# gnosisguild/pvw-rs

Measured on AMD Instinct MI355X. Metric: parties/s for n-party encrypt (pvw::crypto::encrypt); achieved HBM GB/s vs peak, higher is better.
Workload: dtype u64

## Files before the change

### pvw_rs_amd/csrc/pvw_capi.hip

```cpp
#include <hip/hip_runtime.h>

#include <algorithm>
#include <atomic>
#include <cmath>
#include <cstdio>
#include <cstring>
#include <functional>
#include <map>
#include <mutex>
#include <string>
#include <thread>
#include <vector>

#include "../../include/pvw_hip.h"
#include "pvw_arith.h"
#include "pvw_bignum.h"
#include "pvw_chacha.h"
#include "pvw_decode.h"
#include "pvw_kernels.h"
#if PVW_TUNING
#include "../../include/pvw_hip_tuning.h"
#endif

using namespace pvw;
// ... 138 lines not shown
  const bool by_kernel = stream_capturing(s);
  for (const Workspace::Span& sp : w->secrets) {
    hipError_t e = hipSuccess;
    if (!sp.cleared) e = by_kernel && sp.bytes % 8 == 0 ? launch_wipe_words((u64*)sp.p, sp.bytes / 8, s) : hipMemsetAsync(sp.p, 0, sp.bytes, s);
    if (e != hipSuccess) rc = e;
  }
  w->wiped = w->secrets;
  w->secrets.clear();
  return rc;
}

struct pvw_ctx {
  u32 n, k, l, L;
  std::vector<u64> moduli, psi;
  float variance;
  u64 b1, b2;
  u32 num_cus = 256;
  u32 xm_bytes = 8;
  int device;
  u32 party_lo, party_hi, c1_lo, c1_hi;
  BigInt Q, halfQ, delta, delta_pow;
  std::vector<BigInt> crt_qi;
  std::vector<u64> crt_inv;
  std::vector<Mod> mods;
  std::vector<u64> tw, itw, linv, ghat, gpow;
  bool roots_locked = false;
  std::vector<u64> dec_words;
  DecodeTables dec_host{};
  DecodeTables dec_dev{};
  void* d_dec = nullptr;

  std::atomic<bool> dev_ready{false};
  void* d_tables = nullptr;
  DevTables dt{};
  u64* dA = nullptr;
  u64* dB = nullptr;
  u64* xmA = nullptr;
  u64* xmB = nullptr;
  bool xm_valid = false;
  u64* pkA = nullptr;
  u64* pkB = nullptr;
  u32* pk_flag = nullptr;
  u32 pk_width = 0;
  bool pkA_valid = false, pkB_valid = false;
  bool pk_wide = false;
  u32 pk_nomem_calls = 0;
  bool crs_loaded = false;
  u32 num_keys = 0;
  hipStream_t stream = nullptr;

  std::mutex mu, init_mu;
  std::vector<Workspace*> pool;
  std::map<void*, Workspace*> async_ws;

  bool profiling = false;
  std::vector<ProfRec> prof;
  std::map<std::string, std::pair<double, uint64_t>> prof_acc;

  u32 rowsA() const { return c1_hi - c1_lo; }
  u32 rowsB() const { return party_hi - party_lo; }
  u32 R() const { return 128 / l; }
  size_t poly() const { return (size_t)L * l; }
  size_t tiled_words(u32 rows) const { return (size_t)((rows + R() - 1) / R()) * L * k * 128; }
};

struct ProfScope {
  pvw_ctx* c;
  hipStream_t s;
  ProfRec rec;
  bool on;
  ProfScope(pvw_ctx* c_, const char* name, hipStream_t s_) : c(c_), s(s_), on(c_->profiling) {
    if (on) {
      rec.name = name;
      hipEventCreate(&rec.a);
      hipEventCreate(&rec.b);
      hipEventRecord(rec.a, s);
    }
  }
  ~ProfScope() {
    if (on) {
      hipEventRecord(rec.b, s);
      std::lock_guard<std::mutex> g(c->mu);
      c->prof.push_back(rec);
    }
  }
};

static void build_tables(pvw_ctx* c) {
  const u32 L = c->L, l = c->l, bits = ilog2(l);
  c->tw.assign((size_t)L * l, 0);
  c->itw.assign((size_t)L * l, 0);
  c->linv.assign(L, 0);
  c->gpow.assign((size_t)L * l, 0);
  c->ghat.assign((size_t)L * l, 0);
  for (u32 i = 0; i < L; ++i) {
    const Mod& m = c->mods[i];
    u64 psi = c->psi[i], ipsi = powmod(psi, m.q - 2, m);
    for (u32 x = 0; x < l; ++x) {
      c->tw[(size_t)i * l + x] = powmod(psi, bitrev32(x, bits), m);
      c->itw[(size_t)i * l + x] = powmod(ipsi, bitrev32(x, bits), m);
    }
    c->linv[i] = powmod(l, m.q - 2, m);
    u64 dm = c->delta.mod_small(m.q), p = 1;
    for (u32 j = 0; j < l; ++j) {
      c->gpow[(size_t)i * l + j] = p;
      p = mulmod(p, dm, m);
    }
    std::vector<u64> g(c->gpow.begin() + (size_t)i * l, c->gpow.begin() + (size_t)(i + 1) * l);
    host_ntt_forward(g.data(), l, &c->tw[(size_t)i * l], m);
    std::copy(g.begin(), g.end(), c->ghat.begin() + (size_t)i * l);
  }
}

static double correctness_bound(double n, double k, double l, double b1, double b2) {
  double first = b2 * std::sqrt(n * l) * (1.0 + std::sqrt(n));
  double second = 2.0 * b1 * k * l;
  double third = 14.0 * b1 * std::sqrt(n * k * l);
  return first + second + third;
}
// ... 119 lines not shown
  char* p = (char*)c->d_tables;
  auto put = [&](const void* src, size_t n) -> const void* {
    const void* at = p;
    hipMemcpy(p, src, n, hipMemcpyHostToDevice);
    p += n;
    return at;
  };
  c->dt.mods = (const Mod*)put(c->mods.data(), L * sizeof(Mod));
  c->dt.min_q_bits = 64;
  c->dt.max_q_bits = 0;
  for (u32 i = 0; i < L; ++i) {
    u32 bits = 0;
    for (u64 q = c->mods[i].q; q; q >>= 1) ++bits;
    if (bits < c->dt.min_q_bits) c->dt.min_q_bits = bits;
    if (bits > c->dt.max_q_bits) c->dt.max_q_bits = bits;
  }
  c->dt.tw = (const u64*)put(c->tw.data(), L * l * 8);
  c->dt.itw = (const u64*)put(c->itw.data(), L * l * 8);
  c->dt.ghat = (const u64*)put(c->ghat.data(), L * l * 8);
  c->dt.gpow = (const u64*)put(c->gpow.data(), L * l * 8);
  c->dt.linv = (const u64*)put(c->linv.data(), L * 8);
  auto shoup = [&](const std::vector<u64>& src, size_t per_limb) {
    std::vector<u64> out(src.size());
    for (size_t i = 0; i < src.size(); ++i) out[i] = shoup_precompute(src[i], c->moduli[i / per_limb]);
    return out;
  };
  std::vector<u64> twp = shoup(c->tw, l), itwp = shoup(c->itw, l), ghatp = shoup(c->ghat, l),
                   gpowp = shoup(c->gpow, l), linvp = shoup(c->linv, 1);
  c->dt.twp = (const u64*)put(twp.data(), L * l * 8);
  c->dt.itwp = (const u64*)put(itwp.data(), L * l * 8);
  c->dt.ghatp = (const u64*)put(ghatp.data(), L * l * 8);
  c->dt.gpowp = (const u64*)put(gpowp.data(), L * l * 8);
  c->dt.linvp = (const u64*)put(linvp.data(), L * 8);
  if (!c->d_dec) PVW_HIP(hipMalloc(&c->d_dec, c->dec_words.size() * 8));
  PVW_HIP(hipMemcpy(c->d_dec, c->dec_words.data(), c->dec_words.size() * 8, hipMemcpyHostToDevice));
  {
    const u64* hb = c->dec_words.data();
    const u64* db = (const u64*)c->d_dec;
    DecodeTables d = c->dec_host;
    auto mv = [&](const u64* hp) { return db + (hp - hb); };
    d.mods = c->dt.mods;
    d.Q = mv(d.Q); d.halfQ = mv(d.halfQ); d.qi = mv(d.qi); d.inv = mv(d.inv); d.invp = mv(d.invp); d.pow64 = mv(d.pow64);
    d.dmod = mv(d.dmod); d.dmodp = mv(d.dmodp); d.delta = mv(d.delta); d.dpow = mv(d.dpow); d.half_dpow = mv(d.half_dpow);
    d.dpow_n = mv(d.dpow_n); d.td_n = mv(d.td_n);
    d.pow64T = mv(d.pow64T); d.td = mv(d.td); d.mu_td = mv(d.mu_td); d.mu_dp = mv(d.mu_dp); d.gar = mv(d.gar); d.sc = mv(d.sc); d.dpm = mv(d.dpm);
    c->dec_dev = d;
  }
  PVW_HIP(hipDeviceSynchronize());
  return PVW_OK;
}

static int32_t ensure_device(pvw_ctx* c) {
  if (c->dev_ready) {
    PVW_HIP(hipSetDevice(c->device));
    return PVW_OK;
  }
  std::lock_guard<std::mutex> init_guard(c->init_mu);
  if (c->dev_ready) {
    PVW_HIP(hipSetDevice(c->device));
    return PVW_OK;
  }
  int count = 0;
  if (hipGetDeviceCount(&count) != hipSuccess || count == 0)
    return fail(PVW_ERR_INTERNAL, "no HIP device available: the PVW hot path has no CPU fallback");
  if (c->device < 0) {
    int cur = 0;
// ... 411 lines not shown
    c->crt_inv.push_back(powmod(qi.mod_small(c->moduli[i]), c->moduli[i] - 2, c->mods[i]));
  }
  build_tables(c);
  build_decode_tables(c);
  {
    u32 maxbits = 0;
    for (u64 q : c->moduli) {
      u32 bits = 0;
      for (; q; q >>= 1) ++bits;
      if (bits > maxbits) maxbits = bits;
    }
    c->pk_width = packed_width(maxbits, c->k, c->l);
  }
  *out = c;
  return PVW_OK;
}

int32_t pvw_ctx_destroy(pvw_ctx* c) {
  if (!c) return PVW_OK;
  if (c->dev_ready) {
    hipSetDevice(c->device);
    hipDeviceSynchronize();
    for (auto& r : c->prof) { hipEventDestroy(r.a); hipEventDestroy(r.b); }
    for (Workspace* w : c->pool) ws_free(w);
    for (auto& kv : c->async_ws) ws_free(kv.second);
    hipFree(c->dA);
    hipFree(c->dB);
    hipFree(c->xmA);
    hipFree(c->xmB);
    hipFree(c->pkA);
    hipFree(c->pkB);
    hipFree(c->pk_flag);
    hipFree(c->d_tables);
    hipFree(c->d_dec);
    if (c->stream) hipStreamDestroy(c->stream);
  }
  delete c;
  return PVW_OK;
}

int32_t pvw_ctx_get_roots(const pvw_ctx* c, uint64_t* psi_out) {
  if (!c || !psi_out) return fail(PVW_ERR_INVALID_PARAMETERS, "NULL argument");
  memcpy(psi_out, c->psi.data(), c->L * 8);
  return PVW_OK;
}

int32_t pvw_ctx_set_roots(pvw_ctx* c, const uint64_t* psi) {
  if (!c || !psi) return fail(PVW_ERR_INVALID_PARAMETERS, "NULL argument");
  if (c->roots_locked)
    return fail(PVW_ERR_CONTEXT, "roots must be set before any device operation");
  for (u32 i = 0; i < c->L; ++i)
    if (psi[i] >= c->moduli[i] || powmod(psi[i], c->l, c->mods[i]) != c->moduli[i] - 1)
      return fail(PVW_ERR_INVALID_PARAMETERS, "psi is not a primitive 2l-th root of unity");
  c->psi.assign(psi, psi + c->L);
  build_tables(c);
  return PVW_OK;
}

static int32_t export_big(const BigInt& v, uint64_t* words, size_t cap, size_t* nwords) {
  if (!nwords) return fail(PVW_ERR_INVALID_PARAMETERS, "NULL argument");
  *nwords = v.mag.size();
  if (words) {
    if (cap < v.mag.size()) return fail(PVW_ERR_INSUFFICIENT_DATA, "word buffer too small");
    memcpy(words, v.mag.data(), v.mag.size() * 8);
  }
  return PVW_OK;
// ... 1203 lines not shown
      pb.njobs = fused_e2 ? 2 : 3;
      pb.reps = cnt;
      ProfScope ps(c, "prologue", s);
      PVW_HIP(launch_prologue(pb, c->dt, L, l, s));
    }
    u64* c1g = d_c1 + d0 * rA * P;
    u64* c2g = d_c2 + d0 * rB * P;
    const bool last = d0 + nv == D;
    if (use_gemm) {
      {
        ProfScope ps(c, "vec_digits", s);
        PVW_HIP(launch_vec_digits(vh, (size_t)k * P, w->yd, w->sy, nv, k, L, l, c->dt, s, 0, 0, c->xm_bytes));
      }
      ProfScope ps(c, "gemm_digits", s);
      GemmSection a{c->xmA, c1g, c1g, w->gtmpA, rA, 0, 0}, b{c->xmB, c2g, c2g, w->gtmpB, rB, 0, 0};
      std::vector<GemmErrSource> es;
      if (fused_e2) {
        for (u32 v0 = 0; v0 < nv; v0 += PVW_MAX_PROLOGUE_KEYS) {
          GemmErrSource e{};
          e.span = (nv - v0) < PVW_MAX_PROLOGUE_KEYS ? (nv - v0) : PVW_MAX_PROLOGUE_KEYS;
          keys.from(d0 + v0).fill(e, e.span);
          e.key_v = 1;
          e.domain = DOM_E2; e.index0 = c->party_lo; e.index_row = 1; e.index_v = 0; e.bound = c->b2;
          e.scalars = gsc + c->party_lo; e.scalar_v = c->n;
          es.push_back(e);
        }
        b.addend = nullptr;
      }
      if (rs && last) {
        GemmSection& fin = rB ? b : a;
        fin.rnd_ctr = &rs->counter;
        fin.rnd_adv = D;
      }
      PVW_HIP(launch_gemm_digits(a, b, w->yd, w->sy, c->dt, k, L, l, nv, (size_t)rA * P, (size_t)rB * P, s, nullptr, fused_e2 ? es.data() : nullptr, c->xm_bytes));
    } else {
      ProfScope ps(c, "mac_rows_multi", s);
      MacSection a(c->dA, c1g, c1g, rA), b(c->dB, c2g, c2g, rB);
      MultiVec mv{vh, (size_t)k * P, (size_t)rA * P, (size_t)rB * P, nv};
      if (rs && last) {
        a.rnd_ctr = &rs->counter;
        a.rnd_adv = D;
      }
      PVW_HIP(launch_mac_rows_multi(a, b, mv, c->dt, k, L, l, s));
    }
  }
  if (out_repr == PVW_REPR_POWER) {
    ProfScope ps(c, "intt", s);
    PVW_HIP(launch_ntt(d_c1, D * rA, true, c->dt, L, l, s));
    PVW_HIP(launch_ntt(d_c2, D * rB, true, c->dt, L, l, s));
  }
  return PVW_OK;
}

static int32_t encrypt_multi_checks(pvw_ctx* c, size_t D, size_t per_dealer, uint32_t out_repr) {
  PVW_TRY(check_repr(out_repr));
  if (D == 0) return fail(PVW_ERR_INVALID_PARAMETERS, "no dealers");
  if (per_dealer != c->n) {
    char buf[96];
    snprintf(buf, sizeof buf, "Dealer provided %zu shares but needs %u", per_dealer, c->n);
    return fail(PVW_ERR_INVALID_PARAMETERS, buf);
  }
  if (c->num_keys < c->party_hi)
    return fail(PVW_ERR_INVALID_PARAMETERS, "Global public key is not complete (missing party keys)");
  if (!c->crs_loaded) return fail(PVW_ERR_CRS, "CRS not loaded");
  int32_t ok = 0;
  pvw_ctx_verify_correctness_condition(c, &ok);
  if (!ok) return fail(PVW_ERR_INVALID_PARAMETERS, "Parameters do not satisfy correctness condition - decryption may fail");
// ... 1397 lines not shown
  sc.secret(w, r_small0, r_tmp);
  const u32 nchunks = (b - a + chunk - 1) / chunk;
  PVW_TRY(ws_aux(w, 2 * (size_t)nchunks + 2));
  auto upload = [&](u32 ci, hipStream_t st) -> int32_t {
    const u32 q0 = a + ci * chunk, cn = (b - q0) < chunk ? (b - q0) : chunk;
    const size_t wd = (size_t)cn * k * l;
    i64* dst = d_small2[ci & 1];
    PVW_HIP(hipMemcpyAsync(dst, sk + (size_t)(q0 - lo) * k * l, wd * 8, hipMemcpyHostToDevice, st));
    if (ek) PVW_HIP(hipMemcpyAsync(dst + (size_t)chunk * k * l, ek + (size_t)(q0 - lo) * k * l, wd * 8, hipMemcpyHostToDevice, st));
    return PVW_OK;
  };
  PVW_TRY(upload(0, s));
  PVW_HIP(launch_untile(c->dA, d_api, k, 0, k, L, l, false, c->dt, s));
  PVW_HIP(launch_vec_digits(d_api, P, d_yd, d_sy, k, k, L, l, c->dt, s, l, (size_t)k * P));
  for (u32 ci = 0; ci < nchunks; ++ci) {
    const u32 p0 = a + ci * chunk;
    const u32 cnt = (b - p0) < chunk ? (b - p0) : chunk;
    i64* d_small = d_small2[ci & 1];
    if (ci > 0) PVW_HIP(hipStreamWaitEvent(s, w->events[2 * ci], 0));
    ProfScope ps(c, "keygen", s);
    GemmSection ga{d_xm, d_erow, d_erow, d_tmp, cnt, 0, 0}, gb{nullptr, nullptr, nullptr, nullptr, 0, 0, 0};
    ga.tiled_out = c->dB;
    ga.tiled_row0 = p0 - c->party_lo;
    ga.tiled_swap = 1;
    ga.row_stride = (size_t)k * P;
    if (direct) {
      PVW_HIP(launch_shat_mftile(d_small, d_xm, cnt, k, L, l, c->dt, s));
      GemmErrSource es{};
      if (ek) { es.explicit_coeffs = d_small + (size_t)chunk * k * l; es.coef_row = k; es.coef_v = 1; }
      else es.key[0] = make_key(seed);
      es.domain = DOM_EKEY; es.index0 = p0 * k; es.index_row = k; es.index_v = 1; es.bound = c->b1;
      ga.addend = nullptr;
      ga.out = nullptr;
      PVW_HIP(launch_gemm_digits(ga, gb, d_yd, d_sy, c->dt, k, L, l, k, P, 0, s, &es));
    } else {
      PrologueBatch pb{};
      if (seed) pb.key[0] = make_key(seed);
      PrologueJob& js = pb.job[0];
      PrologueJob& je = pb.job[1];
      js.sj.count = k; js.explicit_coeffs = d_small; js.rep_coeffs = (size_t)k * l;
      js.out = d_srow; js.stride_poly = P; js.stride_limb = l; js.rep_out = (size_t)k * P;
      je.sj.kind = SAMPLE_UNIFORM; je.sj.domain = DOM_EKEY; je.sj.index0 = p0 * k; je.sj.count = k; je.sj.bound = c->b1;
      je.rep_index0 = k;
      if (ek) { je.explicit_coeffs = d_small + (size_t)chunk * k * l; je.rep_coeffs = (size_t)k * l; }
      je.out = d_erow; je.stride_poly = P; je.stride_limb = l; je.rep_out = (size_t)k * P;
      pb.njobs = 2;
      pb.reps = cnt;
      PVW_HIP(launch_prologue(pb, c->dt, L, l, s));
      PVW_HIP(hipMemsetAsync(d_xm, 0, xm_words(cnt, k, L, l) * 8, s));
      PVW_HIP(launch_mftile(d_srow, false, d_xm, cnt, k, L, l, s));
      PVW_HIP(launch_gemm_digits(ga, gb, d_yd, d_sy, c->dt, k, L, l, k, P, 0, s));
    }
    PVW_HIP(hipEventRecord(w->events[2 * ci + 1], s));
    if (ci + 1 < nchunks) {
      if (ci >= 1) PVW_HIP(hipStreamWaitEvent(w->aux, w->events[2 * (ci - 1) + 1], 0));
      PVW_TRY(upload(ci + 1, w->aux));
      PVW_HIP(hipEventRecord(w->events[2 * ci + 2], w->aux));
    }
  }
  return PVW_OK;
}

static int32_t keygen_transposed(pvw_ctx* c, Workspace* w, u32 a, u32 b, u32 lo, const int64_t* sk, const int64_t* ek,
                                 const uint8_t* seed, bool use_gemm) {
  const u32 k = c->k, l = c->l, L = c->L;
  const size_t P = c->poly();
  hipStream_t s = w->stream;
// ... 520 lines not shown
```

### pvw_rs_amd/csrc/pvw_gemm.hip

```cpp
#include <hip/hip_runtime.h>

#include "pvw_arith.h"
#include "pvw_chacha.h"
#include "pvw_decode.h"
#include "pvw_kernels.h"
#include "pvw_dev.h"

namespace pvw {

__global__ __launch_bounds__(64) void mfma_i8_probe_kernel(const signed char* __restrict__ A,
                                                            const signed char* __restrict__ B, int* __restrict__ Cm) {
  const u32 l = threadIdx.x, r = l & 31, h = l >> 5;
  union { v4i32 v; signed char b[16]; } fa, fb;
#pragma unroll
  for (int j = 0; j < 16; ++j) {
    fa.b[j] = A[r * 32 + 16 * h + j];
    fb.b[j] = B[(16 * h + j) * 32 + r];
  }
  v16i32 acc = {};
  acc = __builtin_amdgcn_mfma_i32_32x32x32_i8(fa.v, fb.v, acc, 0, 0, 0);
#pragma unroll
  for (int g = 0; g < 16; ++g) Cm[((g & 3) + 8 * (g >> 2) + 4 * h) * 32 + r] = acc[g];
}


template <int ELL>
__global__ __launch_bounds__(256) void mftile_kernel(const u64* __restrict__ src, u32 src_is_tiled,
                                                      u64* __restrict__ XM, u32 rows, u32 k, u32 L) {
  constexpr int R = 128 / ELL;
  const size_t tid = (size_t)blockIdx.x * blockDim.x + threadIdx.x;
  if (tid >= (size_t)rows * k * L) return;
  const u32 limb = tid % L;
  const u32 j = (tid / L) % k;
  const u32 row = tid / ((size_t)L * k);
  const u64* p = src_is_tiled ? src + (((size_t)(row / R) * L + limb) * k + j) * 128 + (row % R) * ELL
                              : src + tid * ELL;
  const u32 RT = ((rows + PVW_GEMM_ROWS_PER_WG - 1) / PVW_GEMM_ROWS_PER_WG) * (PVW_GEMM_ROWS_PER_WG / 32), JB = (k + 3) / 4;
  const u32 rt = row >> 5, m = row & 31, jb = j >> 2, h = (j >> 1) & 1, e = j & 1;
#pragma unroll
// ... 780 lines not shown
    for (int sl = 0; sl < ELL; ++sl) { a[sl] = signed_residue(c[sl], m); x[sl] = in[sl]; }
    if (limb + 1 < limb_end) load_tmp(limb + 1);
    ntt_forward<ELL>(a, t.tw + (size_t)limb * ELL, t.twp + (size_t)limb * ELL, m);
    if (es.scalars) {
      const u64 mr = signed_residue(scalar, m);
      const u64* g = t.ghat + (size_t)limb * ELL;
      const u64* gp = t.ghatp + (size_t)limb * ELL;
#pragma unroll
      for (int sl = 0; sl < ELL; ++sl) a[sl] = addmod(a[sl], mulmod_shoup(mr, g[sl], gp[sl], m.q), m.q);
    }
#pragma unroll
    for (int sl = 0; sl < ELL; sl += 2) {
      const u64 c0 = cbase[((size_t)limb * ELL + sl) * 16], c1 = cbase[((size_t)limb * ELL + sl + 1) * 16];
      *reinterpret_cast<v2u64*>(stg + lane * CST + sl) =
          (v2u64){addmod(addmod(x[sl], a[sl], m.q), c0, m.q), addmod(addmod(x[sl + 1], a[sl + 1], m.q), c1, m.q)};
    }
    __builtin_amdgcn_fence(__ATOMIC_RELEASE, "wavefront");
    __builtin_amdgcn_wave_barrier();
#pragma unroll
    for (int j = 0; j < G; ++j) {
      const v2u64 pv = *reinterpret_cast<const v2u64*>(stg + (gb + j) * CST + 2 * gi);
      const u32 rj = row_raw - gi + j;
      if (rj < sec.nrows && v_ok) {
        const u32 prow = sec.tiled_row0 + rj;
        u64* o = sec.tiled_out ? sec.tiled_out + (((size_t)(prow / R) * L + limb) * nv + v) * 128 + (prow % R) * ELL
                               : sec.out + (size_t)v * ostride + (size_t)rj * rstride + (size_t)limb * ELL;
        *reinterpret_cast<v2u64*>(o + 2 * gi) = pv;
      }
    }
    __builtin_amdgcn_fence(__ATOMIC_RELEASE, "wavefront");
    __builtin_amdgcn_wave_barrier();
  }
}
hipError_t launch_mftile(const u64* src, bool src_is_tiled, u64* XM, u32 rows, u32 k, u32 L, u32 ell, hipStream_t s, u32 bytes,
                         const Mod* mods) {
  if (rows == 0) return hipSuccess;
  if (bytes == 7) {
    if (!mods) return hipErrorInvalidValue;
    const u32 RT = ((rows + PVW_GEMM_ROWS_PER_WG - 1) / PVW_GEMM_ROWS_PER_WG) * (PVW_GEMM_ROWS_PER_WG / 32);
    const size_t threads = (size_t)RT * 32 * L * ell * (k / 32) * 2;
    PVW_DISPATCH_ELL(ell, mftile7_kernel<E><<<dim3((u32)((threads + 255) / 256)), dim3(256), 0, s>>>(src, src_is_tiled ? 1u : 0u, XM, rows, k, L, mods));
    return hipGetLastError();
  }
  if (!src_is_tiled && ell <= 32) {
    const u32 jbg = ell <= 8 ? 4 : (ell == 16 ? 2 : 1);
    const u32 JB = (k + 3) / 4, JG = (JB + jbg - 1) / jbg;
    const u32 RT = ((rows + PVW_GEMM_ROWS_PER_WG - 1) / PVW_GEMM_ROWS_PER_WG) * (PVW_GEMM_ROWS_PER_WG / 32);
    switch (ell) {
      case 8: mftile_rows_kernel<8><<<dim3(JG * RT * L), dim3(256), 0, s>>>(src, XM, rows, k, L); break;
      case 16: mftile_rows_kernel<16><<<dim3(JG * RT * L), dim3(256), 0, s>>>(src, XM, rows, k, L); break;
      default: mftile_rows_kernel<32><<<dim3(JG * RT * L), dim3(256), 0, s>>>(src, XM, rows, k, L); break;
    }
    return hipGetLastError();
  }
  const size_t threads = (size_t)rows * k * L;
  PVW_DISPATCH_ELL(ell, mftile_kernel<E><<<dim3((u32)((threads + 255) / 256)), dim3(256), 0, s>>>(src, src_is_tiled ? 1u : 0u, XM, rows, k, L));
  return hipGetLastError();
}

hipError_t launch_shat_mftile(const i64* coeffs, u64* XM, u32 rows, u32 k, u32 L, u32 ell, const DevTables& t, hipStream_t s) {
  if (rows == 0) return hipSuccess;
  if (ell > 32) return hipErrorInvalidValue;
  const u32 jbg = 2;
  const u32 JB = (k + 3) / 4, JG = (JB + jbg - 1) / jbg;
  const u32 RT = ((rows + PVW_GEMM_ROWS_PER_WG - 1) / PVW_GEMM_ROWS_PER_WG) * (PVW_GEMM_ROWS_PER_WG / 32);
  u32 ls = 1;
// ... 52 lines not shown
    else { PVW_DISPATCH_ELL(ell, gemm_digits_kernel<E, G, PVW_GEMM_RPW, N, false><<<dim3(blocks * vbn), dim3(256), 0, s>>>(sa, sb, YD, SY, t.mods, k, L, nv, nv_pad, vbn, yd_b16, sy_b16, kt)); } \
  } while (0)
#if PVW_TUNING
  if (PVW_ENV_INT("PVW_GEMM_ZERO_OPERANDS", 0)) {
    if (sa.nrows) (void)hipMemsetAsync(const_cast<u64*>(sa.XM), 0, xm_words(sa.nrows, k, L, ell) * 8, s);
    if (sb.nrows) (void)hipMemsetAsync(const_cast<u64*>(sb.XM), 0, xm_words(sb.nrows, k, L, ell) * 8, s);
    (void)hipMemsetAsync(const_cast<signed char*>(YD), 0, yd_b16 * vbn, s);
  }
#endif
  const bool wide = vbn >= 2 && k % 16 == 0 && k >= 16 && kt % 2 == 0 && PVW_ENV_INT("PVW_GEMM_WIDE", 1) != 0;
  if (wide) {
    const u32 ga = (sa.rt_groups * 4 + 7) / 8, gb2 = (sb.rt_groups * 4 + 7) / 8;
    const u32 wblocks = (ga + gb2) * L * ell * ((vbn + 1) / 2);
    if (t.min_q_bits >= 55) { PVW_DISPATCH_ELL(ell, gemm_digits_wide_kernel<E, true><<<dim3(wblocks), dim3(512), 0, s>>>(sa, sb, YD, t.mods, k, L, nv, nv_pad, vbn, yd_b16, kt)); }
    else { PVW_DISPATCH_ELL(ell, gemm_digits_wide_kernel<E, false><<<dim3(wblocks), dim3(512), 0, s>>>(sa, sb, YD, t.mods, k, L, nv, nv_pad, vbn, yd_b16, kt)); }
  } else {
  static const int unroll_ok = (int)PVW_ENV_INT("PVW_GEMM_UNROLL", 1);
  if (NVG == 4 && unroll_ok && kt == 64) { PVW_GEMM_LAUNCH(4, 8); }
  else if (NVG == 4 && unroll_ok && kt == 128) { PVW_GEMM_LAUNCH(4, 16); }
  else switch (NVG) {
    case 1: PVW_GEMM_LAUNCH(1, 0); break;
    case 2: PVW_GEMM_LAUNCH(2, 0); break;
    case 3: PVW_GEMM_LAUNCH(3, 0); break;
    case 4: PVW_GEMM_LAUNCH(4, 0); break;
    default: return hipErrorInvalidValue;
  }
#undef PVW_GEMM_LAUNCH
  }
  return hipGetLastError();
}

hipError_t launch_gemm_digits(const GemmSection& a, const GemmSection& b, const signed char* YD, const int* SY,
                              const DevTables& t, u32 k, u32 L, u32 ell, u32 nv, size_t ostride_a, size_t ostride_b,
                              hipStream_t s, const GemmErrSource* es_a, const GemmErrSource* es_b, u32 bytes) {
  GemmSection sa = a, sb = b;
  if ((sa.nrows == 0 && sb.nrows == 0) || nv == 0) return hipSuccess;
  {
    const hipError_t ge = launch_gemm_digits_core(sa, sb, YD, SY, t, k, L, ell, nv, s, bytes);
    if (ge != hipSuccess) return ge;
  }
  const u32 vbn = (nv + 15) / 16;
  const u32 nv_pad = (vbn > 1 ? 4 : (nv + 3) / 4) * 4;
  const size_t sy_b16 = sy_bytes(16, L, ell) / sizeof(int);
  auto finish = [&](const GemmSection& sec, size_t ostride, const GemmErrSource* es) -> hipError_t {
    if (!sec.nrows) return hipSuccess;
    const u32 rows_pad = sec.rt_groups * PVW_GEMM_ROWS_PER_WG;
    if (es) {
      if (ell > 32 || (sec.tiled_out && !sec.tiled_swap) || (!sec.tiled_out && !sec.out)) return hipErrorInvalidValue;
      for (u32 v_lo = 0; v_lo < nv; ++es) {
        const u32 span = es->span && es->span < nv - v_lo ? es->span : nv - v_lo, v_hi = v_lo + span;
        GemmSection sec_l = sec;
        if (v_hi < nv) sec_l.rnd_ctr = nullptr;
        const u32 gx = (sec.nrows + 31) / 32;
        bool one_wave = false;
#if PVW_TUNING
        one_wave = PVW_ENV_INT("PVW_FINISH_VPB", 8) == 2;
        if (one_wave) {
          const dim3 grid(gx, (span + 1) / 2, 1);
          switch (ell) {
            case 8: gemm_finish_err_kernel<8, 2><<<grid, dim3(64), 0, s>>>(sec_l, t, L, nv, nv_pad, rows_pad, ostride, SY, sy_b16, *es, v_lo, v_hi); break;
            case 16: gemm_finish_err_kernel<16, 2><<<grid, dim3(64), 0, s>>>(sec_l, t, L, nv, nv_pad, rows_pad, ostride, SY, sy_b16, *es, v_lo, v_hi); break;
            default: gemm_finish_err_kernel<32, 2><<<grid, dim3(64), 0, s>>>(sec_l, t, L, nv, nv_pad, rows_pad, ostride, SY, sy_b16, *es, v_lo, v_hi); break;
          }
        }
#endif
        if (!one_wave) {
          const u32 gy = (span + 7) / 8;
          u32 lz = 1;
          const size_t want = (size_t)PVW_ENV_INT("PVW_FINISH_BLOCKS", 4096);
          while (lz < L && (size_t)gx * gy * lz < want) lz *= 2;
          if (lz > L) lz = L;
          const dim3 grid(gx, gy, lz);
          switch (ell) {
            case 8: gemm_finish_err_kernel<8, 8><<<grid, dim3(256), 0, s>>>(sec_l, t, L, nv, nv_pad, rows_pad, ostride, SY, sy_b16, *es, v_lo, v_hi); break;
            case 16: gemm_finish_err_kernel<16, 8><<<grid, dim3(256), 0, s>>>(sec_l, t, L, nv, nv_pad, rows_pad, ostride, SY, sy_b16, *es, v_lo, v_hi); break;
            default: gemm_finish_err_kernel<32, 8><<<grid, dim3(256), 0, s>>>(sec_l, t, L, nv, nv_pad, rows_pad, ostride, SY, sy_b16, *es, v_lo, v_hi); break;
          }
        }
        v_lo = v_hi;
      }
      return hipGetLastError();
    }
    PVW_DISPATCH_ELL(ell, gemm_finish_kernel<E><<<dim3((sec.nrows + 31) / 32, (nv + (E >= 64 ? 2 : 4) - 1) / (E >= 64 ? 2 : 4), L), dim3(256), 0, s>>>(
                              sec, t.mods, L, nv, nv_pad, rows_pad, ostride, SY, sy_b16));
    return hipGetLastError();
  };
// ... 84 lines not shown
```

### pvw_rs_amd/csrc/pvw_kernels.h

```cpp
#pragma once
#include <hip/hip_runtime.h>

#include "pvw_arith.h"
#include "pvw_chacha.h"
#include "pvw_decode.h"

#ifndef PVW_TUNING
#define PVW_TUNING 0
#endif
#if PVW_TUNING
#include <cstdlib>
#define PVW_ENV_INT(name, dflt) ([]() -> long { const char* e_ = getenv(name); return e_ ? atol(e_) : (long)(dflt); }())
#else
#define PVW_ENV_INT(name, dflt) ((long)(dflt))
#endif

namespace pvw {

enum { DOM_R = 0, DOM_E1 = 1, DOM_E2 = 2, DOM_SK = 3, DOM_EKEY = 4, DOM_CRS = 5, DOM_GAUSS = 6, DOM_PK = 7, DOM_CALL = 8 };

struct RndState {
  u32 seed[8];
  u64 counter;
  u64 base;
};
PVW_HD ChaChaKey call_seed(const u32 seed[8], u64 c) {
  ChaChaKey k;
#pragma unroll
  for (int i = 0; i < 8; ++i) k.w[i] = seed[i];
  ChaChaRng g;
  g.init(k, DOM_CALL, 0);
  g.counter = c;
  g.refill();
#pragma unroll
  for (int i = 0; i < 8; ++i) k.w[i] = g.buf[i];
  return k;
}
__device__ __forceinline__ void rnd_advance(u64* ctr, u64 adv) {
  if (ctr && blockIdx.x == 0 && blockIdx.y == 0 && blockIdx.z == 0 && threadIdx.x == 0) *ctr += adv;
}

struct DevTables {
  const Mod* mods;
  const u64* tw;
  const u64* itw;
  const u64* linv;
  const u64* ghat;
  const u64* gpow;
  const u64* twp;
  const u64* itwp;
  const u64* linvp;
  const u64* ghatp;
  const u64* gpowp;
  u32 min_q_bits;
  u32 max_q_bits;
};

enum { SAMPLE_CBD = 0, SAMPLE_UNIFORM = 1 };
struct SampleJob {
  u32 kind;
  u32 domain;
  u32 index0;
  u32 count;
  u32 out_poly0;
  u32 cbd_half;
  u32 cbd_v;
  u64 bound;
};

struct MacSection {
  const u64* M = nullptr;
  const u64* addend = nullptr;
  u64* out = nullptr;
  u32 nrows = 0;
  u32 row_blocks = 0;
  MacSection() = default;
  MacSection(const u64* M_, const u64* addend_, u64* out_, u32 nrows_) : M(M_), addend(addend_), out(out_), nrows(nrows_) {}
  const i64* e_small = nullptr;
  const u64* scalars = nullptr;
  u64* rnd_ctr = nullptr;
  u64 rnd_adv = 0;
};
hipError_t launch_prep(const i64* coeffs, const u64* scalars, u64* out, size_t stride_poly,
                       size_t stride_limb, u32 count, bool do_ntt, const DevTables& t, u32 L,
                       u32 ell, hipStream_t s, u32 group = 0, size_t stride_group = 0);
hipError_t launch_transpose_polys(const u64* src, u64* dst, u32 k, u32 words, hipStream_t s);
// ... 133 lines not shown
  u64 rnd_adv = 0;
};
inline size_t gemm_tmp_words(u32 rows, u32 L, u32 ell) {
  return (size_t)L * ell * 16 * (((rows + PVW_GEMM_ROWS_PER_WG - 1) / PVW_GEMM_ROWS_PER_WG) * PVW_GEMM_ROWS_PER_WG);
}
inline size_t xm_words(u32 rows, u32 k, u32 L, u32 ell) {
  return (size_t)L * ell * (((rows + PVW_GEMM_ROWS_PER_WG - 1) / PVW_GEMM_ROWS_PER_WG) * (PVW_GEMM_ROWS_PER_WG / 32)) *
         ((k + 3) / 4) * 128;
}
inline size_t yd_bytes(u32 nv, u32 k, u32 L, u32 ell) { return (size_t)((nv + 3) / 4) * L * ell * ((k + 3) / 4) * 1024; }
inline u32 gemm_ktiles(u32 k, u32 bytes) { return bytes == 7 ? 7 * (k / 32) : (k + 3) / 4; }
inline bool gemm7_ok(u32 max_q_bits, u32 k) { return max_q_bits <= 56 && k % 64 == 0 && k >= 64; }
inline size_t sy_bytes(u32 nv, u32 L, u32 ell) { return (size_t)((nv + 3) / 4) * L * ell * 32 * sizeof(int); }
hipError_t launch_mftile(const u64* src, bool src_is_tiled, u64* XM, u32 rows, u32 k, u32 L, u32 ell, hipStream_t s, u32 bytes = 8,
                         const Mod* mods = nullptr);
hipError_t launch_shat_mftile(const i64* coeffs, u64* XM, u32 rows, u32 k, u32 L, u32 ell, const DevTables& t, hipStream_t s);
hipError_t launch_vec_digits(const u64* vhat, size_t vstride, signed char* YD, int* SY, u32 nv, u32 k, u32 L, u32 ell,
                             const DevTables& t, hipStream_t s, size_t lstride = 0, size_t jstride = 0, u32 bytes = 8);
struct GemmErrSource {
  u32 span;
  const i64* explicit_coeffs;
  size_t coef_row, coef_v;
  ChaChaKey key[PVW_MAX_PROLOGUE_KEYS];
  u32 key_v;
  u32 domain, index0, index_row, index_v;
  u64 bound;
  const u64* scalars;
  size_t scalar_v;
  const RndState* rnd;
  u64 rnd_off;
};
hipError_t launch_gemm_digits(const GemmSection& a, const GemmSection& b, const signed char* YD, const int* SY,
                              const DevTables& t, u32 k, u32 L, u32 ell, u32 nv, size_t ostride_a, size_t ostride_b,
                              hipStream_t s, const GemmErrSource* es_a = nullptr, const GemmErrSource* es_b = nullptr, u32 bytes = 8);
hipError_t launch_gemm_digits_core(GemmSection& a, GemmSection& b, const signed char* YD, const int* SY, const DevTables& t, u32 k,
                                   u32 L, u32 ell, u32 nv, hipStream_t s, u32 bytes = 8);
hipError_t launch_finish_decrypt(const GemmSection& a, const int* SY, const DevTables& t, u32 L, u32 ell, u32 nv, const u64* c2,
                                 size_t c2_vstride, size_t c2_rstride, u64* noisy, hipStream_t s);
hipError_t launch_reduce_words(const u64* src, u64* dst, size_t words, const DevTables& t, u32 L, u32 ell, hipStream_t s);
#if PVW_TUNING
hipError_t read_stamps(u64* out, u32* hw, u32 count);
hipError_t init_probe_attributes();
hipError_t launch_read_probe(const u64* M, size_t total_tiles, u32 tiles_per_wave, u64* sink, hipStream_t s);
hipError_t launch_read_probe2(const u64* M, size_t total_tiles, u32 tiles_per_wave, u64* sink, u32 U, bool dbuf, u32 lds_bytes,
                              hipStream_t s, u32 xmap = 0);
#endif
hipError_t init_kernel_attributes();
hipError_t launch_mfma_probe(const signed char* A, const signed char* B, int* C, hipStream_t s);
hipError_t launch_decode(u64* noisy, u64* out, size_t count, const DecodeTables& t, hipStream_t s, const DevTables* xf = nullptr,
                         u64* wipe = nullptr, size_t wipe_bytes = 0, bool* wiped = nullptr, u64* noise = nullptr,
                         u32* status = nullptr, const PlainArgs* plain = nullptr);

hipError_t launch_wire_pack(const u64* words, size_t count, unsigned char* out, const Mod* mods, u32 L, u32 ell, hipStream_t s);
hipError_t launch_wire_unpack(const unsigned char* in, size_t count, u64* words, unsigned long long* bad, const Mod* mods, u32 L,
                              u32 ell, hipStream_t s);
hipError_t init_wire_attributes();

}
```

Measured before the change: 22.24 million.

## Compute GEMM finish error-NTT and scalar terms with int8 MFMA via precomputed tables

Adds a precomputed per-limb table of byte-split NTT basis vectors and ghat powers, and a new finish kernel. The kernel samples the uniform error polynomial, splits it and the scalar into signed byte digits, and evaluates the forward NTT plus the scalar-times-ghat term as int8 MFMA products against the table. Results are recombined modulo q with a fast float-quotient path or a 128-bit fallback. This replaces per-thread scalar NTT arithmetic in the fused-e2 finish stage with matrix-core work, at the cost of extra table memory, LDS staging and a bound restriction on the error magnitude.

```diff
diff --git a/pvw_rs_amd/csrc/pvw_capi.hip b/pvw_rs_amd/csrc/pvw_capi.hip
--- a/pvw_rs_amd/csrc/pvw_capi.hip
+++ b/pvw_rs_amd/csrc/pvw_capi.hip
@@ -194,6 +194,7 @@
 
   std::atomic<bool> dev_ready{false};
   void* d_tables = nullptr;
+  void* d_fintab = nullptr;
   DevTables dt{};
   u64* dA = nullptr;
   u64* dB = nullptr;
@@ -247,6 +248,12 @@
     }
   }
 };
+
+static void prof_count(pvw_ctx* c, const char* name, u32 n) {
+  if (!c->profiling || !n) return;
+  std::lock_guard<std::mutex> g(c->mu);
+  c->prof_acc[name].second += n;
+}
 
 static void build_tables(pvw_ctx* c) {
   const u32 L = c->L, l = c->l, bits = ilog2(l);
@@ -432,6 +439,12 @@
   c->dt.ghatp = (const u64*)put(ghatp.data(), L * l * 8);
   c->dt.gpowp = (const u64*)put(gpowp.data(), L * l * 8);
   c->dt.linvp = (const u64*)put(linvp.data(), L * 8);
+  c->dt.fintab = nullptr;
+  if (const size_t fb = finish_table_bytes((u32)L, (u32)l)) {
+    if (!c->d_fintab) PVW_HIP(hipMalloc(&c->d_fintab, fb));
+    PVW_HIP(launch_finish_table(c->dt, (u32)L, (u32)l, c->d_fintab, nullptr));
+    c->dt.fintab = c->d_fintab;
+  }
   if (!c->d_dec) PVW_HIP(hipMalloc(&c->d_dec, c->dec_words.size() * 8));
   PVW_HIP(hipMemcpy(c->d_dec, c->dec_words.data(), c->dec_words.size() * 8, hipMemcpyHostToDevice));
   {
@@ -909,6 +922,7 @@
     hipFree(c->pkB);
     hipFree(c->pk_flag);
     hipFree(c->d_tables);
+    hipFree(c->d_fintab);
     hipFree(c->d_dec);
     if (c->stream) hipStreamDestroy(c->stream);
   }
@@ -2178,7 +2192,10 @@
         fin.rnd_ctr = &rs->counter;
         fin.rnd_adv = D;
       }
-      PVW_HIP(launch_gemm_digits(a, b, w->yd, w->sy, c->dt, k, L, l, nv, (size_t)rA * P, (size_t)rB * P, s, nullptr, fused_e2 ? es.data() : nullptr, c->xm_bytes));
+      u32 mfma_finishes = 0;
+      PVW_HIP(launch_gemm_digits(a, b, w->yd, w->sy, c->dt, k, L, l, nv, (size_t)rA * P, (size_t)rB * P, s, nullptr, fused_e2 ? es.data() : nullptr, c->xm_bytes,
+                                 &mfma_finishes));
+      prof_count(c, "finish_mfma", mfma_finishes);
     } else {
       ProfScope ps(c, "mac_rows_multi", s);
       MacSection a(c->dA, c1g, c1g, rA), b(c->dB, c2g, c2g, rB);
@@ -3642,7 +3659,9 @@
       es.domain = DOM_EKEY; es.index0 = p0 * k; es.index_row = k; es.index_v = 1; es.bound = c->b1;
       ga.addend = nullptr;
       ga.out = nullptr;
-      PVW_HIP(launch_gemm_digits(ga, gb, d_yd, d_sy, c->dt, k, L, l, k, P, 0, s, &es));
+      u32 mfma_finishes = 0;
+      PVW_HIP(launch_gemm_digits(ga, gb, d_yd, d_sy, c->dt, k, L, l, k, P, 0, s, &es, nullptr, 8, &mfma_finishes));
+      prof_count(c, "finish_mfma", mfma_finishes);
     } else {
       PrologueBatch pb{};
       if (seed) pb.key[0] = make_key(seed);
diff --git a/pvw_rs_amd/csrc/pvw_finish_digits.h b/pvw_rs_amd/csrc/pvw_finish_digits.h
--- /dev/null
+++ b/pvw_rs_amd/csrc/pvw_finish_digits.h
@@ -0,0 +1,19 @@
+#pragma once
+#include "pvw_arith.h"
+
+namespace pvw {
+
+constexpr u64 PVW_FINISH_ERR_MAX = 32639;
+constexpr u32 PVW_FINISH_SCALAR_DIGITS = 9;
+
+PVW_HD u32 finish_err_digits(i64 e) { return (((u32)(int32_t)e + 0x8080u) ^ 0x8080u) & 0xffffu; }
+
+PVW_HD u32 finish_scalar_digits(u64 u, u64& low) {
+  const u64 C = 0x8080808080808080ULL;
+  const u64 t = u + C;
+  low = t ^ C;
+  const int d8 = (int)(t < u) - (int)(u >> 63);
+  return (u32)d8 & 0xffu;
+}
+
+}
diff --git a/pvw_rs_amd/csrc/pvw_gemm.hip b/pvw_rs_amd/csrc/pvw_gemm.hip
--- a/pvw_rs_amd/csrc/pvw_gemm.hip
+++ b/pvw_rs_amd/csrc/pvw_gemm.hip
@@ -5,6 +5,7 @@
 #include "pvw_decode.h"
 #include "pvw_kernels.h"
 #include "pvw_dev.h"
+#include "pvw_finish_digits.h"
 
 namespace pvw {
 
@@ -851,6 +852,226 @@
     __builtin_amdgcn_wave_barrier();
   }
 }
+__host__ __device__ constexpr u32 finish_ks(u32 ell) { return (2 * ell + PVW_FINISH_SCALAR_DIGITS + 31) / 32; }
+__host__ __device__ constexpr u32 finish_slot(u32 ell, u32 t, u32 s4) { return (s4 >> 1) * (ell / 2) + 2 * t + (s4 & 1); }
+size_t finish_table_bytes(u32 L, u32 ell) { return ell == 8 || ell == 16 ? (size_t)L * (ell / 4) * finish_ks(ell) * 1024 : 0; }
+
+template <int ELL>
+__global__ __launch_bounds__(64) void finish_table_kernel(DevTables t, v4i32* __restrict__ tab) {
+  constexpr u32 T = ELL / 4, KS = finish_ks(ELL);
+  const u32 lane = threadIdx.x, h = lane >> 5, s4 = (lane & 31) >> 3, b = lane & 7;
+  const u32 ks = blockIdx.x % KS, tt = (blockIdx.x / KS) % T, limb = blockIdx.x / (KS * T);
+  const Mod m = t.mods[limb];
+  const u32 slot = finish_slot(ELL, tt, s4);
+  u64 w256, w256p;
+  mul256_consts(m, w256, w256p);
+  union { v4i32 v; unsigned char by[16]; } f;
+#pragma unroll 1
+  for (u32 p = 0; p < 16; ++p) {
+    const u32 kap = 32 * ks + 16 * h + p;
+    u64 w = 0;
+    u32 shifts = 0;
+    if (kap < 2 * ELL) {
+      u64 a[ELL];
+#pragma unroll
+      for (int sl = 0; sl < ELL; ++sl) a[sl] = (u32)sl == (kap >> 1) ? 1 : 0;
+      ntt_forward<ELL>(a, t.tw + (size_t)limb * ELL, t.twp + (size_t)limb * ELL, m);
+#pragma unroll
+      for (int sl = 0; sl < ELL; ++sl) w = (u32)sl == slot ? a[sl] : w;
+      shifts = kap & 1;
+    } else if (kap < 2 * ELL + PVW_FINISH_SCALAR_DIGITS) {
+      w = reduce_word(t.ghat[(size_t)limb * ELL + slot], m);
+      shifts = kap - 2 * ELL;
+    }
+    for (u32 a = 0; a < shifts; ++a) w = mulmod_shoup(w, w256, w256p, m.q);
+    const u64 C = 0x8080808080808080ULL;
+    f.by[p] = (unsigned char)(((w + C) ^ C) >> (8 * b));
+  }
+  tab[(((size_t)limb * T + tt) * KS + ks) * 64 + lane] = f.v;
+}
+hipError_t launch_finish_table(const DevTables& t, u32 L, u32 ell, void* tab, hipStream_t s) {
+  if (!finish_table_bytes(L, ell)) return hipErrorInvalidValue;
+  const dim3 grid(L * (ell / 4) * finish_ks(ell));
+  if (ell == 8) finish_table_kernel<8><<<grid, dim3(64), 0, s>>>(t, reinterpret_cast<v4i32*>(tab));
+  else finish_table_kernel<16><<<grid, dim3(64), 0, s>>>(t, reinterpret_cast<v4i32*>(tab));
+  return hipGetLastError();
+}
+
+template <bool FASTQ>
+__device__ __forceinline__ void finish_recombine(const v16i32& a, const Mod& m, double inv32, u64 (&res)[2]) {
+  int lo[4], hi[4];
+#pragma unroll
+  for (int s4 = 0; s4 < 4; ++s4) {
+    lo[s4] = a[4 * s4] + a[4 * s4 + 1] * 256;
+    hi[s4] = a[4 * s4 + 2] + a[4 * s4 + 3] * 256;
+  }
+#pragma unroll
+  for (int pr = 0; pr < 2; ++pr) {
+    const auto sl = __builtin_amdgcn_permlane32_swap((u32)lo[pr], (u32)lo[pr + 2], false, false);
+    const auto sh = __builtin_amdgcn_permlane32_swap((u32)hi[pr], (u32)hi[pr + 2], false, false);
+    const int ll = (int)sl[0], hl = (int)sl[1], lh = (int)sh[0], hh = (int)sh[1];
+    const i64 lo4 = (i64)ll + (i64)lh * 65536, hi4 = (i64)hl + (i64)hh * 65536;
+    if constexpr (FASTQ) {
+      const double dh = __builtin_fma((double)hh, 65536.0, (double)hl);
+      const int qhat = (int)(dh * inv32);
+      i64 s = (i64)(((u64)hi4 << 32) - (u64)(i64)qhat * m.q) + lo4;
+      if (s < 0) s += (i64)m.q;
+      if (s < 0) s += (i64)m.q;
+      if (s >= (i64)m.q) s -= (i64)m.q;
+      res[pr] = (u64)s;
+    } else {
+      const __int128 tot = (__int128)lo4 + ((__int128)hi4 << 32);
+      u64 l = (u64)tot, hw = (u64)((unsigned __int128)tot >> 64);
+      const bool neg = (long long)hw < 0;
+      if (neg) { l = ~l + 1; hw = ~hw + (l == 0); }
+      u64 r = reduce128(l, hw, m);
+      if (neg && r) r = m.q - r;
+      res[pr] = r;
+    }
+  }
+}
+
+template <int ELL, bool FASTQ>
+__global__ __launch_bounds__(256, ELL == 8 ? 4 : 2) void gemm_finish_mfma_kernel(GemmSection sec, DevTables t, u32 L, u32 nv, u32 nv_pad, u32 rows_pad,
+                                                                size_t ostride, const int* __restrict__ SY, size_t sy_b16, GemmErrSource es,
+                                                                u32 v_lo, u32 v_hi) {
+  constexpr int T = ELL / 4, KS = (int)finish_ks(ELL), HS = ELL / 2, VPB = 8;
+  constexpr bool PF = ELL == 8;
+  constexpr int G = ELL / 2, RPI = 64 / G, NI = 32 / RPI;
+  constexpr int CST = ELL + 2;
+  __shared__ v4i32 frag[VPB / 2][2 * KS * 64];
+  __shared__ u64 stage[VPB / 2][32 * CST];
+  __shared__ ChaChaKey vkey[VPB];
+  const u32 tid = threadIdx.x, lane = tid & 63, wave = __builtin_amdgcn_readfirstlane(tid >> 6), h = lane >> 5, rr = lane & 31;
+  const u32 row_raw = blockIdx.x * 32 + rr;
+  const u32 row = row_raw < sec.nrows ? row_raw : sec.nrows - 1;
+  rnd_advance(sec.rnd_ctr, sec.rnd_adv);
+  {
+    const u32 v_raw = v_lo + blockIdx.y * VPB + (tid >> 5);
+    const u32 v = v_raw < v_hi ? v_raw : v_hi - 1;
+    if (es.rnd) {
+      if (rr == 0) vkey[tid >> 5] = call_seed(es.rnd->seed, es.rnd->base + es.rnd_off + (u64)(v - v_lo) * es.key_v);
+      __builtin_amdgcn_fence(__ATOMIC_RELEASE, "wavefront");
+      __builtin_amdgcn_wave_barrier();
+      __builtin_amdgcn_fence(__ATOMIC_ACQUIRE, "wavefront");
+    }
+    unsigned char* fb = reinterpret_cast<unsigned char*>(&frag[wave][0]);
+    ChaChaRng g;
+    g.init(es.rnd ? vkey[tid >> 5] : es.key[(v - v_lo) * es.key_v], es.domain, es.index0 + row * es.index_row + v * es.index_v);
+    auto emit = [fb, h, rr](u32 sl, i64 val) {
+      const u32 kap = 2 * sl;
+      *reinterpret_cast<unsigned short*>(fb + (((h * KS + (kap >> 5)) * 64 + ((kap >> 4) & 1) * 32 + rr) * 16 + (kap & 15))) =
+          (unsigned short)finish_err_digits(val);
+    };
+    sample_uniform_poly(g, ELL, es.bound, emit);
+    u64 low;
+    const u32 d8 = finish_scalar_digits(es.scalars ? es.scalars[(size_t)v * es.scalar_v + row] : 0, low);
+    constexpr u32 kap0 = 2 * ELL;
+    frag[wave][(h * KS + (kap0 >> 5)) * 64 + ((kap0 >> 4) & 1) * 32 + rr] = (v4i32){(int)(u32)low, (int)(u32)(low >> 32), (int)d8, 0};
+    if constexpr (ELL == 16) frag[wave][(h * KS + 1) * 64 + 32 + rr] = (v4i32){0, 0, 0, 0};
+    __builtin_amdgcn_fence(__ATOMIC_RELEASE, "wavefront");
+    __builtin_amdgcn_wave_barrier();
+    __builtin_amdgcn_fence(__ATOMIC_ACQUIRE, "wavefront");
+  }
+  v4i32 bf[2][KS];
+#pragma unroll
+  for (int tile = 0; tile < 2; ++tile)
+#pragma unroll
+    for (int ks = 0; ks < KS; ++ks) bf[tile][ks] = frag[wave][(tile * KS + ks) * 64 + lane];
+  constexpr u32 R = 128 / ELL;
+  const size_t rstride = sec.row_stride ? sec.row_stride : (size_t)L * ELL;
+  const size_t sstride = (size_t)nv_pad * rows_pad;
+  const size_t lstride = sec.tiled_out ? (size_t)nv * 128 : (size_t)ELL;
+  const u64* tbase[2];
+  const u64* cbase[2];
+  u64* obase[2];
+  bool ok[2];
+#pragma unroll
+  for (int tile = 0; tile < 2; ++tile) {
+    const u32 v_raw = v_lo + blockIdx.y * VPB + wave * 2 + tile;
+    const u32 v = v_raw < v_hi ? v_raw : v_hi - 1;
+    ok[tile] = v_raw < v_hi;
+    tbase[tile] = sec.tmp + (v >> 4) * sec.tmp_bstride + (size_t)(nv_pad == 16 ? (v & 15) : v) * rows_pad + row + (size_t)(h * HS) * sstride;
+    cbase[tile] = reinterpret_cast<const u64*>(SY + (size_t)(v >> 4) * sy_b16 + ((size_t)((v & 15) >> 2) * L * ELL) * 32) + (v & 3) + (size_t)(h * HS) * 16;
+    obase[tile] = sec.tiled_out ? sec.tiled_out + (size_t)v * 128 : sec.out + (size_t)v * ostride;
+  }
+  const u32 gi = lane % G;
+  size_t rowoff[NI];
+  bool rowok[NI];
+#pragma unroll
+  for (int i = 0; i < NI; ++i) {
+    const u32 rj = blockIdx.x * 32 + lane / G + RPI * i;
+    const u32 prow = sec.tiled_row0 + rj;
+    rowok[i] = rj < sec.nrows;
+    rowoff[i] = (sec.tiled_out ? (size_t)(prow / R) * L * nv * 128 + (prow % R) * ELL : (size_t)rj * rstride) + 2 * gi;
+  }
+  u64* stg = stage[wave];
+  const v4i32* tab = reinterpret_cast<const v4i32*>(t.fintab) + lane;
+  u64 in[2][HS], cin[2][HS];
+  v4i32 tf[T][KS];
+  auto load_small = [&](u32 limb) {
+#pragma unroll
+    for (int tile = 0; tile < 2; ++tile)
+#pragma unroll
+      for (int j = 0; j < HS; ++j) cin[tile][j] = cbase[tile][((size_t)limb * ELL + j) * 16];
+#pragma unroll
+    for (int tt = 0; tt < T; ++tt)
+#pragma unroll
+      for (int ks = 0; ks < KS; ++ks) tf[tt][ks] = tab[(((size_t)limb * T + tt) * KS + ks) * 64];
+  };
+  auto load_limb = [&](u32 limb) {
+#pragma unroll
+    for (int tile = 0; tile < 2; ++tile)
+#pragma unroll
+      for (int j = 0; j < HS; ++j) in[tile][j] = __builtin_nontemporal_load(tbase[tile] + ((size_t)limb * ELL + j) * sstride);
+    if constexpr (PF) load_small(limb);
+  };
+  const u32 per = (L + gridDim.z - 1) / gridDim.z, limb_end = (blockIdx.z + 1) * per < L ? (blockIdx.z + 1) * per : L;
+  u32 limb = blockIdx.z * per;
+  if (limb < limb_end) load_limb(limb);
+  for (; limb < limb_end; ++limb) {
+    const Mod m = t.mods[limb];
+    const double inv32 = gemm_inv32(m, false);
+    u64 x[2][HS];
+    v4i32 tc[T][KS];
+    if constexpr (!PF) load_small(limb);
+#pragma unroll
+    for (int tile = 0; tile < 2; ++tile)
+#pragma unroll
+      for (int j = 0; j < HS; ++j) x[tile][j] = addmod(in[tile][j], cin[tile][j], m.q);
+#pragma unroll
+    for (int tt = 0; tt < T; ++tt)
+#pragma unroll
+      for (int ks = 0; ks < KS; ++ks) tc[tt][ks] = tf[tt][ks];
+    load_limb(limb + 1 < limb_end ? limb + 1 : limb);
+#pragma unroll
+    for (int tile = 0; tile < 2; ++tile) {
+#pragma unroll
+      for (int tt = 0; tt < T; ++tt) {
+        v16i32 acc = gemm_acc_init(false);
+#pragma unroll
+        for (int ks = 0; ks < KS; ++ks) acc = __builtin_amdgcn_mfma_i32_32x32x32_i8(tc[tt][ks], bf[tile][ks], acc, 0, 0, 0);
+        u64 res[2];
+        finish_recombine<FASTQ>(acc, m, inv32, res);
+        x[tile][2 * tt] = addmod(x[tile][2 * tt], res[0], m.q);
+        x[tile][2 * tt + 1] = addmod(x[tile][2 * tt + 1], res[1], m.q);
+      }
+#pragma unroll
+      for (int j = 0; j < HS; j += 2) *reinterpret_cast<v2u64*>(stg + rr * CST + h * HS + j) = (v2u64){x[tile][j], x[tile][j + 1]};
+      __builtin_amdgcn_fence(__ATOMIC_RELEASE, "wavefront");
+      __builtin_amdgcn_wave_barrier();
+      __builtin_amdgcn_fence(__ATOMIC_ACQUIRE, "wavefront");
+#pragma unroll
+      for (int i = 0; i < NI; ++i) {
+        const v2u64 pv = *reinterpret_cast<const v2u64*>(stg + (lane / G + RPI * i) * CST + 2 * gi);
+        if (ok[tile] && rowok[i]) *reinterpret_cast<v2u64*>(obase[tile] + rowoff[i] + (size_t)limb * lstride) = pv;
+      }
+      __builtin_amdgcn_fence(__ATOMIC_RELEASE, "wavefront");
+      __builtin_amdgcn_wave_barrier();
+    }
+  }
+}
+
 hipError_t launch_mftile(const u64* src, bool src_is_tiled, u64* XM, u32 rows, u32 k, u32 L, u32 ell, hipStream_t s, u32 bytes,
                          const Mod* mods) {
   if (rows == 0) return hipSuccess;
@@ -969,7 +1190,7 @@
 
 hipError_t launch_gemm_digits(const GemmSection& a, const GemmSection& b, const signed char* YD, const int* SY,
                               const DevTables& t, u32 k, u32 L, u32 ell, u32 nv, size_t ostride_a, size_t ostride_b,
-                              hipStream_t s, const GemmErrSource* es_a, const GemmErrSource* es_b, u32 bytes) {
+                              hipStream_t s, const GemmErrSource* es_a, const GemmErrSource* es_b, u32 bytes, u32* mfma_finishes) {
   GemmSection sa = a, sb = b;
   if ((sa.nrows == 0 && sb.nrows == 0) || nv == 0) return hipSuccess;
   {
@@ -989,6 +1210,23 @@
         GemmSection sec_l = sec;
         if (v_hi < nv) sec_l.rnd_ctr = nullptr;
         const u32 gx = (sec.nrows + 31) / 32;
+        if ((ell == 8 || ell == 16) && !es->explicit_coeffs && es->bound <= PVW_FINISH_ERR_MAX && t.fintab &&
+            PVW_ENV_INT("PVW_FINISH_MFMA", 1) != 0) {
+          const u32 gy = (span + 7) / 8;
+          u32 lz = 1;
+          while (lz < L && (size_t)gx * gy * lz < 512) lz *= 2;
+          if (lz > L) lz = L;
+          const dim3 grid(gx, gy, lz);
+          const bool fastq = t.min_q_bits >= 55;
+#define PVW_FINISH_MFMA_LAUNCH(E, F) \
+  gemm_finish_mfma_kernel<E, F><<<grid, dim3(256), 0, s>>>(sec_l, t, L, nv, nv_pad, rows_pad, ostride, SY, sy_b16, *es, v_lo, v_hi)
+          if (ell == 8) { if (fastq) PVW_FINISH_MFMA_LAUNCH(8, true); else PVW_FINISH_MFMA_LAUNCH(8, false); }
+          else { if (fastq) PVW_FINISH_MFMA_LAUNCH(16, true); else PVW_FINISH_MFMA_LAUNCH(16, false); }
+#undef PVW_FINISH_MFMA_LAUNCH
+          if (mfma_finishes) ++*mfma_finishes;
+          v_lo = v_hi;
+          continue;
+        }
         bool one_wave = false;
 #if PVW_TUNING
         one_wave = PVW_ENV_INT("PVW_FINISH_VPB", 8) == 2;
diff --git a/pvw_rs_amd/csrc/pvw_kernels.h b/pvw_rs_amd/csrc/pvw_kernels.h
--- a/pvw_rs_amd/csrc/pvw_kernels.h
+++ b/pvw_rs_amd/csrc/pvw_kernels.h
@@ -52,6 +52,7 @@
   const u64* linvp;
   const u64* ghatp;
   const u64* gpowp;
+  const void* fintab;
   u32 min_q_bits;
   u32 max_q_bits;
 };
@@ -251,7 +252,10 @@
 };
 hipError_t launch_gemm_digits(const GemmSection& a, const GemmSection& b, const signed char* YD, const int* SY,
                               const DevTables& t, u32 k, u32 L, u32 ell, u32 nv, size_t ostride_a, size_t ostride_b,
-                              hipStream_t s, const GemmErrSource* es_a = nullptr, const GemmErrSource* es_b = nullptr, u32 bytes = 8);
+                              hipStream_t s, const GemmErrSource* es_a = nullptr, const GemmErrSource* es_b = nullptr, u32 bytes = 8,
+                              u32* mfma_finishes = nullptr);
+size_t finish_table_bytes(u32 L, u32 ell);
+hipError_t launch_finish_table(const DevTables& t, u32 L, u32 ell, void* tab, hipStream_t s);
 hipError_t launch_gemm_digits_core(GemmSection& a, GemmSection& b, const signed char* YD, const int* SY, const DevTables& t, u32 k,
                                    u32 L, u32 ell, u32 nv, hipStream_t s, u32 bytes = 8);
 hipError_t launch_finish_decrypt(const GemmSection& a, const int* SY, const DevTables& t, u32 L, u32 ell, u32 nv, const u64* c2,
```

Result: slower. 21.46 million (-3.5%).
